# pettni/smooth_feedback

Measured on AMD Instinct MI355X. Metric: QP solves/sec, higher is better.
Workload: dtype f64

## Files before the change

include/sfb.h:

```cpp
#ifndef SFB_H
#define SFB_H

#include <stdint.h>

#ifdef __cplusplus
extern "C" {
#endif

typedef enum sfb_status {
  SFB_OK              = 0,
  SFB_ERR_INVALID_ARG = 1,
  SFB_ERR_UNSUPPORTED = 2,
  SFB_ERR_HIP         = 3,
  SFB_ERR_NO_DEVICE   = 4
} sfb_status;

typedef enum sfb_qp_status {
  SFB_QP_OPTIMAL           = 0,
  SFB_QP_POLISH_FAILED     = 1,
  SFB_QP_PRIMAL_INFEASIBLE = 2,
  SFB_QP_DUAL_INFEASIBLE   = 3,
  SFB_QP_MAX_ITERATIONS    = 4,
  SFB_QP_MAX_TIME          = 5,
  SFB_QP_UNKNOWN           = 6
// ... 64 lines not shown
                                         const double *P, const double *q, const double *A, const double *l,
                                         const double *u, const double *warm_x, const double *warm_y,
                                         double *x, double *y, double *obj, uint32_t *iter, int32_t *code);
void sfb_host_staging_trim(void);
sfb_status sfb_qp_dense_solve_batch_host_trace(const sfb_qp_params *prm, int64_t batch, int n, int m, const double *P,
                                               const double *q, const double *A, const double *l, const double *u,
                                               const double *warm_x, const double *warm_y, double *x, double *y, double *obj,
                                               uint32_t *iter, int32_t *code, double *trace, int32_t trace_rows);
sfb_status sfb_qp_dense_solve_batch_host_phases(const sfb_qp_params *prm, int64_t batch, int n, int m, const double *P,
                                                const double *q, const double *A, const double *l, const double *u,
                                                const double *warm_x, const double *warm_y, double *x, double *y, double *obj,
                                                uint32_t *iter, int32_t *code, double *trace, int32_t trace_rows,
                                                double *phase_us);
sfb_status sfb_qp_dense_solve_batch_host_multi(const sfb_qp_params *prm, int64_t batch, int n, int m,
                                               const double *P, const double *q, const double *A, const double *l,
                                               const double *u, const double *warm_x, const double *warm_y,
                                               double *x, double *y, double *obj, uint32_t *iter, int32_t *code);

#define SFB_QP_DENSE_TALL_MAX_N 16
#define SFB_QP_DENSE_TALL_MAX_M 1048576
sfb_status sfb_qp_dense_tall_solve_batch(const sfb_qp_params *prm, int64_t batch, int n, int m, const double *P,
                                         const double *q, const double *A, const double *l, const double *u,
                                         const double *warm_x, const double *warm_y, double *x, double *y,
                                         double *obj, uint32_t *iter, int32_t *code, void *stream);
sfb_status sfb_qp_dense_tall_solve_batch_host(const sfb_qp_params *prm, int64_t batch, int n, int m,
                                              const double *P, const double *q, const double *A, const double *l,
                                              const double *u, const double *warm_x, const double *warm_y,
                                              double *x, double *y, double *obj, uint32_t *iter, int32_t *code);
sfb_status sfb_qp_dense_tall_solve_batch_host_multi(const sfb_qp_params *prm, int64_t batch, int n, int m,
                                                    const double *P, const double *q, const double *A, const double *l,
                                                    const double *u, const double *warm_x, const double *warm_y,
                                                    double *x, double *y, double *obj, uint32_t *iter, int32_t *code);

typedef struct sfb_sparse_qp_plan sfb_sparse_qp_plan;

sfb_status sfb_sparse_qp_plan_create(int n, int m, const int32_t *P_colptr, const int32_t *P_rowind,
                                     const int32_t *A_rowptr, const int32_t *A_colind, int ordering,
                                     const int32_t *user_perm, sfb_sparse_qp_plan **plan);
sfb_status sfb_sparse_qp_plan_create_staged(int n, int m, const int32_t *P_colptr, const int32_t *P_rowind,
                                            const int32_t *A_rowptr, const int32_t *A_colind, int ordering,
                                            const int32_t *user_perm, const int32_t *stage,
                                            sfb_sparse_qp_plan **plan);
sfb_status sfb_sparse_qp_plan_create_pruned(int n, int m, const int32_t *P_colptr, const int32_t *P_rowind,
                                            const int32_t *A_rowptr, const int32_t *A_colind, int ordering,
                                            const int32_t *user_perm, const int32_t *stage, const uint8_t *A_keep,
                                            sfb_sparse_qp_plan **plan);
void sfb_sparse_qp_plan_destroy(sfb_sparse_qp_plan *plan);
sfb_status sfb_sparse_qp_plan_info(const sfb_sparse_qp_plan *plan, int64_t *nnzK, int64_t *nnzL,
                                   int64_t *workspace_bytes_per_item);
sfb_status sfb_sparse_qp_plan_workspace_bytes(const sfb_sparse_qp_plan *plan, int64_t batch, int64_t *bytes);
sfb_status sfb_sparse_qp_plan_pruned_info(const sfb_sparse_qp_plan *plan, int64_t *nnzA_kept, int64_t *nnzL_fallback);
sfb_status sfb_sparse_qp_plan_get_perm(const sfb_sparse_qp_plan *plan, int32_t *perm);
sfb_status sfb_sparse_qp_plan_get_factor_order(const sfb_sparse_qp_plan *plan, int fallback, int32_t *rank);

sfb_status sfb_sparse_qp_solve_batch(sfb_sparse_qp_plan *plan, const sfb_qp_params *prm, int64_t batch,
                                     const double *Px, const double *q, const double *Ax, const double *l,
                                     const double *u, const double *warm_x, const double *warm_y, double *x,
                                     double *y, double *obj, uint32_t *iter, int32_t *code, void *workspace,
                                     void *stream);
sfb_status sfb_sparse_qp_solve_batch_ordered(sfb_sparse_qp_plan *plan, const sfb_qp_params *prm, int64_t batch,
                                             const double *Px, const double *q, const double *Ax, const double *l,
                                             const double *u, const double *warm_x, const double *warm_y, double *x,
                                             double *y, double *obj, uint32_t *iter, int32_t *code, void *workspace,
                                             const int32_t *order, void *stream);
sfb_status sfb_sparse_qp_solve_batch_trace(sfb_sparse_qp_plan *plan, const sfb_qp_params *prm, int64_t batch,
                                           const double *Px, const double *q, const double *Ax, const double *l,
                                           const double *u, const double *warm_x, const double *warm_y, double *x,
                                           double *y, double *obj, uint32_t *iter, int32_t *code, void *workspace,
                                           double *trace, int32_t trace_rows, void *stream);
sfb_status sfb_sparse_qp_solve_batch_phases(sfb_sparse_qp_plan *plan, const sfb_qp_params *prm, int64_t batch,
                                            const double *Px, const double *q, const double *Ax, const double *l,
                                            const double *u, const double *warm_x, const double *warm_y, double *x,
                                            double *y, double *obj, uint32_t *iter, int32_t *code, void *workspace,
                                            double *trace, int32_t trace_rows, double *phase_us, void *stream);
sfb_status sfb_sparse_qp_solve_batch_host(sfb_sparse_qp_plan *plan, const sfb_qp_params *prm, int64_t batch,
                                          const double *Px, const double *q, const double *Ax, const double *l,
                                          const double *u, const double *warm_x, const double *warm_y,
                                          double *x, double *y, double *obj, uint32_t *iter, int32_t *code);
sfb_status sfb_sparse_qp_solve_batch_host_trace(sfb_sparse_qp_plan *plan, const sfb_qp_params *prm, int64_t batch,
                                                const double *Px, const double *q, const double *Ax, const double *l,
                                                const double *u, const double *warm_x, const double *warm_y, double *x,
                                                double *y, double *obj, uint32_t *iter, int32_t *code, double *trace,
                                                int32_t trace_rows);
sfb_status sfb_sparse_qp_solve_batch_host_phases(sfb_sparse_qp_plan *plan, const sfb_qp_params *prm, int64_t batch,
                                                 const double *Px, const double *q, const double *Ax, const double *l,
                                                 const double *u, const double *warm_x, const double *warm_y,
                                                 double *x, double *y, double *obj, uint32_t *iter, int32_t *code,
                                                 double *trace, int32_t trace_rows, double *phase_us);
sfb_status sfb_sparse_qp_solve_batch_host_multi(sfb_sparse_qp_plan *plan, const sfb_qp_params *prm, int64_t batch,
                                                const double *Px, const double *q, const double *Ax, const double *l,
                                                const double *u, const double *warm_x, const double *warm_y,
                                                double *x, double *y, double *obj, uint32_t *iter, int32_t *code);

typedef enum { SFB_LIE_RN = 0, SFB_LIE_SE2 = 1, SFB_LIE_SO3 = 2, SFB_LIE_SE3 = 3 } sfb_lie_kind;

typedef struct sfb_mpc_layout {
  int32_t nx, nu, ncr;
  int32_t kmesh, nivals;
  double tf;
  const double *alpha;
  const double *D;
  int32_t nparts;
  const int32_t *part_kind;
  const int32_t *part_dof;
  const double *crl, *cru;
  const uint8_t *jac_keep;
// ... 167 lines not shown
```

smooth_feedback_amd/_capi.py:

```python
import ctypes as C
import os

_HERE = os.path.dirname(os.path.abspath(__file__))
LIB_PATH = os.environ.get("SFB_LIB_PATH") or os.path.join(_HERE, "libsfb.so")

SFB_OK, SFB_ERR_INVALID_ARG, SFB_ERR_UNSUPPORTED, SFB_ERR_HIP, SFB_ERR_NO_DEVICE = range(5)


class SfbError(RuntimeError):
    def __init__(self, status, msg):
        super().__init__("sfb status %d: %s" % (status, msg))
        self.status = status


class SfbQPParams(C.Structure):

    _fields_ = [
        ("alpha", C.c_float),
        ("rho", C.c_float),
        ("sigma", C.c_float),
        ("scaling", C.c_int32),
        ("eps_abs", C.c_float),
        ("eps_rel", C.c_float),
        ("eps_primal_inf", C.c_float),
# ... 29 lines not shown
    _fields_ = [("nivals", C.c_int32), ("K", C.c_void_p), ("tau0", C.c_void_p)]


class SfbOcpDims(C.Structure):

    _fields_ = [("nx", C.c_int32), ("nu", C.c_int32), ("nq", C.c_int32), ("ncr", C.c_int32), ("nce", C.c_int32)]


def _load():
    if not os.path.exists(LIB_PATH):
        raise ImportError(
            "libsfb.so not found at %s: build it with `python -c 'import __graft_entry__ as g; g.build()'` "
            "or `make -C smooth_feedback_amd/csrc` (there is no CPU fallback)" % LIB_PATH)
    try:
        import torch
    except Exception:
        pass
    L = C.CDLL(LIB_PATH)
    vp, dp, i64, i32 = C.c_void_p, C.c_void_p, C.c_int64, C.c_int
    L.sfb_version.restype = C.c_char_p
    L.sfb_last_error.restype = C.c_char_p
    L.sfb_debug_set.argtypes = [C.c_char_p, C.c_char_p]
    L.sfb_device_count.argtypes = [C.POINTER(C.c_int)]
    L.sfb_qp_params_default.argtypes = [C.POINTER(SfbQPParams)]
    L.sfb_qp_params_default.restype = None
    L.sfb_qp_dense_solve_batch.argtypes = [C.POINTER(SfbQPParams), i64, i32, i32] + [dp] * 12 + [vp]
    L.sfb_qp_dense_solve_batch_host.argtypes = [C.POINTER(SfbQPParams), i64, i32, i32] + [dp] * 12
    L.sfb_qp_dense_solve_batch_host_multi.argtypes = L.sfb_qp_dense_solve_batch_host.argtypes
    L.sfb_qp_dense_tall_solve_batch.argtypes = L.sfb_qp_dense_solve_batch.argtypes
    L.sfb_qp_dense_tall_solve_batch_host.argtypes = L.sfb_qp_dense_solve_batch_host.argtypes
    L.sfb_qp_dense_tall_solve_batch_host_multi.argtypes = L.sfb_qp_dense_solve_batch_host.argtypes
    L.sfb_qp_dense_solve_batch_host_trace.argtypes = [C.POINTER(SfbQPParams), i64, i32, i32] + [dp] * 12 + [dp, i32]
    L.sfb_qp_dense_solve_batch_trace.argtypes = [C.POINTER(SfbQPParams), i64, i32, i32] + [dp] * 12 + [dp, i32, vp]
    L.sfb_qp_dense_solve_batch_host_phases.argtypes = [C.POINTER(SfbQPParams), i64, i32, i32] + [dp] * 12 + [dp, i32, dp]
    L.sfb_qp_dense_solve_batch_phases.argtypes = [C.POINTER(SfbQPParams), i64, i32, i32] + [dp] * 12 + [dp, i32, dp, vp]
    L.sfb_qp_dense_solve_batch_ws.argtypes = [C.POINTER(SfbQPParams), i64, i32, i32] + [dp] * 12 + [vp, vp]
    L.sfb_qp_dense_workspace_bytes.argtypes = [C.POINTER(SfbQPParams), i64, i32, i32, C.POINTER(C.c_int64)]
    L.sfb_workspace_create.argtypes = [i64, C.POINTER(C.c_void_p)]
    L.sfb_workspace_destroy.argtypes = [C.c_void_p]
    L.sfb_workspace_destroy.restype = None
    L.sfb_workspace_info.argtypes = [C.c_void_p, C.POINTER(C.c_void_p), C.POINTER(C.c_int64)]
    i32p = C.c_void_p
    L.sfb_sparse_qp_plan_create.argtypes = [i32, i32, i32p, i32p, i32p, i32p, i32, i32p, C.POINTER(C.c_void_p)]
    L.sfb_sparse_qp_plan_create_staged.argtypes = [i32, i32, i32p, i32p, i32p, i32p, i32, i32p, i32p, C.POINTER(C.c_void_p)]
    L.sfb_sparse_qp_plan_create_pruned.argtypes = [i32, i32, i32p, i32p, i32p, i32p, i32, i32p, i32p, C.c_void_p,
                                                   C.POINTER(C.c_void_p)]
    L.sfb_sparse_qp_plan_workspace_bytes.argtypes = [C.c_void_p, i64, C.POINTER(C.c_int64)]
    L.sfb_sparse_qp_plan_pruned_info.argtypes = [C.c_void_p, C.POINTER(C.c_int64), C.POINTER(C.c_int64)]
    L.sfb_sparse_qp_plan_destroy.argtypes = [C.c_void_p]
    L.sfb_sparse_qp_plan_destroy.restype = None
    L.sfb_sparse_qp_plan_info.argtypes = [C.c_void_p, C.POINTER(C.c_int64), C.POINTER(C.c_int64), C.POINTER(C.c_int64)]
    L.sfb_sparse_qp_plan_get_perm.argtypes = [C.c_void_p, i32p]
    L.sfb_sparse_qp_plan_get_factor_order.argtypes = [C.c_void_p, i32, i32p]
    L.sfb_sparse_qp_solve_batch.argtypes = [C.c_void_p, C.POINTER(SfbQPParams), i64] + [dp] * 12 + [vp, vp]
    L.sfb_sparse_qp_solve_batch_ordered.argtypes = [C.c_void_p, C.POINTER(SfbQPParams), i64] + [dp] * 12 + [vp, vp, vp]
    L.sfb_sparse_qp_solve_batch_host.argtypes = [C.c_void_p, C.POINTER(SfbQPParams), i64] + [dp] * 12
    L.sfb_sparse_qp_solve_batch_host_multi.argtypes = L.sfb_sparse_qp_solve_batch_host.argtypes
    L.sfb_sparse_qp_solve_batch_host_trace.argtypes = [C.c_void_p, C.POINTER(SfbQPParams), i64] + [dp] * 12 + [dp, i32]
    L.sfb_sparse_qp_solve_batch_trace.argtypes = [C.c_void_p, C.POINTER(SfbQPParams), i64] + [dp] * 12 + [vp, dp, i32, vp]
    L.sfb_sparse_qp_solve_batch_host_phases.argtypes = [C.c_void_p, C.POINTER(SfbQPParams), i64] + [dp] * 12 + [dp, i32, dp]
    L.sfb_sparse_qp_solve_batch_phases.argtypes = [C.c_void_p, C.POINTER(SfbQPParams), i64] + [dp] * 12 + [vp, dp, i32, dp, vp]
    L.sfb_ekf_predict_batch.argtypes = [i64, i32, dp, dp, i32, dp, i32, dp, vp]
    L.sfb_ekf_predict_stepper_batch.argtypes = [i32, i64, i32, dp, dp, i32, dp, i32, dp, vp]
    L.sfb_ekf_predict_stepper_batch_host.argtypes = [i32, i64, i32, dp, dp, i32, dp, i32, dp]
    L.sfb_ekf_predict_rk4_batch.argtypes = [i64, i32, dp, dp, dp, dp, i32, dp, i32, dp, vp]
    L.sfb_ekf_predict_rk4_batch_host.argtypes = [i64, i32, dp, dp, dp, dp, i32, dp, i32, dp]
    L.sfb_ekf_update_batch.argtypes = [i64, i32, i32, dp, dp, i32, dp, dp, dp, dp, vp]
    L.sfb_ekf_predict_update_batch.argtypes = [i64, i32, i32, dp, dp, i32, dp, i32, dp, dp, i32, dp, dp, dp, dp, vp]
    L.sfb_ekf_step_batch_host.argtypes = [i64, i32, i32, dp, dp, i32, dp, i32, dp, dp, i32, dp, dp, dp, dp]
    grp, dbl = C.POINTER(SfbPIDGroup), C.c_double
    L.sfb_pid_elem_doubles.argtypes = [grp]
    L.sfb_pid_elem_doubles.restype = i64
    L.sfb_pid_dof.argtypes = [grp]
    L.sfb_pid_dof.restype = i64
    L.sfb_pid_step_batch_host.argtypes = [grp, i64, dbl] + [dp] * 5 + [i32] + [dp] * 3 + [i32, dbl] + [dp] * 3
    L.sfb_pid_step_batch.argtypes = L.sfb_pid_step_batch_host.argtypes + [vp]
    L.sfb_pid_rollout_batch_host.argtypes = [grp, i64, dbl, dbl, i64] + [dp] * 4 + [i32] + [dp] * 3 + [i32, dbl] + [dp] * 5
    L.sfb_pid_rollout_batch.argtypes = L.sfb_pid_rollout_batch_host.argtypes + [vp]
    L.sfb_spline_fit_cubic_batch_host.argtypes = [grp, i64, i64, dp, i32, dp, dp]
    L.sfb_spline_fit_cubic_batch.argtypes = L.sfb_spline_fit_cubic_batch_host.argtypes + [vp]
    L.sfb_spline_eval_batch_host.argtypes = [grp, i64, i64, dp, dp, dp, i32, dp, i64, dp, i32, dp, dp, dp]
    L.sfb_spline_eval_batch.argtypes = L.sfb_spline_eval_batch_host.argtypes + [vp]
    L.sfb_pid_rollout_spline_batch_host.argtypes = [grp, i64, dbl, dbl, i64, dp, dp, i64, dp, dp, dp, i32, dp] + [dp] * 3 + [i32, dbl] + [dp] * 5
    L.sfb_pid_rollout_spline_batch.argtypes = L.sfb_pid_rollout_spline_batch_host.argtypes + [vp]
    mesh = C.POINTER(SfbMesh)
    L.sfb_mesh_raised_nodes.argtypes = [mesh, dp]
    L.sfb_mesh_resample_batch_host.argtypes = [mesh, i64, i32, i32, dp, dp]
    L.sfb_mesh_resample_batch.argtypes = L.sfb_mesh_resample_batch_host.argtypes + [vp]
    L.sfb_mesh_dyn_error_batch_host.argtypes = [mesh, i64, i32, dp, dp, dp, dp]
    L.sfb_mesh_dyn_error_batch.argtypes = L.sfb_mesh_dyn_error_batch_host.argtypes + [vp]
    L.sfb_mesh_eval_pattern.argtypes = [mesh, i32, i32, i32, vp, vp, C.POINTER(C.c_int64)]
    L.sfb_mesh_dyn_pattern.argtypes = [mesh, i32, i32, vp, vp, C.POINTER(C.c_int64)]
    L.sfb_mesh_eval_batch_host.argtypes = [mesh, i64, i32, i32, i32, i32] + [dp] * 6
    L.sfb_mesh_eval_batch.argtypes = L.sfb_mesh_eval_batch_host.argtypes + [vp]
    L.sfb_mesh_integrate_batch_host.argtypes = [mesh, i64, i32, i32, i32] + [dp] * 6
    L.sfb_mesh_integrate_batch.argtypes = L.sfb_mesh_integrate_batch_host.argtypes + [vp]
    L.sfb_mesh_dyn_batch_host.argtypes = [mesh, i64, i32, i32] + [dp] * 7
    L.sfb_mesh_dyn_batch.argtypes = L.sfb_mesh_dyn_batch_host.argtypes + [vp]
    dims = C.POINTER(SfbOcpDims)
    L.sfb_ocp_nlp_structure.argtypes = [mesh, dims, vp, vp]
    L.sfb_ocp_nlp_pattern.argtypes = [mesh, dims, vp, vp, C.POINTER(C.c_int64)]
    L.sfb_ocp_nlp_bounds.argtypes = [mesh, dims] + [dp] * 8 + [C.POINTER(C.c_double)]
    L.sfb_ocp_nlp_batch_host.argtypes = [mesh, dims, i64] + [dp] * 11
    L.sfb_ocp_nlp_batch.argtypes = L.sfb_ocp_nlp_batch_host.argtypes + [vp]
    lay = C.POINTER(SfbMPCLayout)
    L.sfb_mpc_record_doubles.argtypes = [lay, i32]
# ... 61 lines not shown
```

smooth_feedback_amd/csrc/capi_sparse.hip:

```cpp
#include <hip/hip_runtime.h>

#include <algorithm>
#include <chrono>
#include <cstdio>
#include <map>
#include <mutex>
#include <string>
#include <vector>

#include "../../include/sfb.h"
#include "capi_common.h"
#include "qp_sparse_kernel.h"
#include "sparse_plan.h"

struct sfb_sparse_qp_plan {
  sfb::SparsePlanHost host;
  bool pruned = false;
  sfb::SparsePlanHost full;
  std::vector<int32_t> Aorig, Amasked;
  std::mutex mu;
  struct DevCopy {
    int32_t *blob = nullptr, *blob_full = nullptr;
    sfb::SparsePlanDev dev{}, dev_full{};
  };
// ... 227 lines not shown
  for (auto &kv : plan->per_device) {
    if (kv.second.blob) (void)hipFree(kv.second.blob);
    if (kv.second.blob_full) (void)hipFree(kv.second.blob_full);
  }
  for (auto &kv : plan->host_dev) {
    if (kv.second.ws.first) (void)hipFree(kv.second.ws.first);
    if (kv.second.stream) (void)hipStreamDestroy(kv.second.stream);
    if (kv.second.uploaded) (void)hipEventDestroy(kv.second.uploaded);
  }
  delete plan;
}

sfb_status sfb_sparse_qp_plan_info(const sfb_sparse_qp_plan *plan, int64_t *nnzK, int64_t *nnzL,
                                   int64_t *workspace_bytes_per_item)
{
  if (!plan) return sfb::fail(SFB_ERR_INVALID_ARG, "plan is NULL");
  if (nnzK) *nnzK = plan->host.nnzK;
  if (nnzL) *nnzL = plan->host.nnzL;
  if (workspace_bytes_per_item) {
    const WsLayout L1 = ws_layout(plan, 1);
    *workspace_bytes_per_item = (int64_t)L1.total;
  }
  return SFB_OK;
}

sfb_status sfb_sparse_qp_plan_workspace_bytes(const sfb_sparse_qp_plan *plan, int64_t batch, int64_t *bytes)
{
  if (!plan || !bytes) return sfb::fail(SFB_ERR_INVALID_ARG, "NULL argument");
  if (batch < 0) return sfb::fail(SFB_ERR_INVALID_ARG, "batch < 0");
  *bytes = (int64_t)ws_layout(plan, batch).total;
  return SFB_OK;
}

sfb_status sfb_sparse_qp_plan_pruned_info(const sfb_sparse_qp_plan *plan, int64_t *nnzA_kept, int64_t *nnzL_fallback)
{
  if (!plan) return sfb::fail(SFB_ERR_INVALID_ARG, "plan is NULL");
  if (nnzA_kept) *nnzA_kept = plan->host.nnzA;
  if (nnzL_fallback) *nnzL_fallback = plan->pruned ? plan->full.nnzL : plan->host.nnzL;
  return SFB_OK;
}

sfb_status sfb_sparse_qp_plan_get_perm(const sfb_sparse_qp_plan *plan, int32_t *perm)
{
  if (!plan || !perm) return sfb::fail(SFB_ERR_INVALID_ARG, "NULL argument");
  std::copy(plan->host.perm.begin(), plan->host.perm.end(), perm);
  return SFB_OK;
}

sfb_status sfb_sparse_qp_plan_get_factor_order(const sfb_sparse_qp_plan *plan, int fallback, int32_t *rank)
{
  if (!plan || !rank) return sfb::fail(SFB_ERR_INVALID_ARG, "NULL argument");
  const sfb::SparsePlanHost &h = (fallback && plan->pruned) ? plan->full : plan->host;
  for (int f = 0; f < h.k; ++f) rank[h.f2s[f]] = f;
  return SFB_OK;
}

namespace {
sfb_status solve_batch_impl(sfb_sparse_qp_plan *plan, const sfb_qp_params *prm, int64_t batch,
                                     const double *Px, const double *q, const double *Ax, const double *l,
                                     const double *u, const double *warm_x, const double *warm_y, double *x,
                                     double *y, double *obj, uint32_t *iter, int32_t *code, void *workspace,
                                             const int32_t *order, void *stream, double *trace, int32_t trace_rows,
                                             double *phase_us = nullptr)
{
  sfb_status st = check_sparse_args(plan, prm, batch, Px, q, Ax, l, u, warm_x, warm_y, x, y, code);
  if (st != SFB_OK) return st;
  if (batch > 0 && !workspace) return sfb::fail(SFB_ERR_INVALID_ARG, "workspace is NULL");
  st = sfb::require_device();
  if (st != SFB_OK) return st;
  if (batch == 0) return SFB_OK;
  const sfb_sparse_qp_plan::DevCopy *dc = nullptr;
  st = plan_on_device(plan, &dc);
  if (st != SFB_OK) return st;
  const sfb::DenseKernelParams kp = sfb::make_kernel_params(prm, plan->host.n, plan->host.m);
  hipStream_t hs   = static_cast<hipStream_t>(stream);
  const WsLayout L = ws_layout(plan, batch);
  char *wsc        = static_cast<char *>(workspace);
  hipError_t e     = sfb::qp_sparse_launch(dc->dev, kp, batch, Px, q, Ax, l, u, warm_x, warm_y, x, y, obj, iter, code,
                                           reinterpret_cast<double *>(wsc), hs, order, reinterpret_cast<int32_t *>(wsc + L.aux_off),
                                           plan->pruned ? &dc->dev_full : nullptr, reinterpret_cast<double *>(wsc + L.pool_off),
                                           trace, (int)trace_rows, phase_us);
  if (e != hipSuccess) return sfb::hip_fail(e, "qp_sparse_kernel launch");
  return SFB_OK;
}
}

sfb_status sfb_sparse_qp_solve_batch_ordered(sfb_sparse_qp_plan *plan, const sfb_qp_params *prm, int64_t batch,
                                             const double *Px, const double *q, const double *Ax, const double *l,
                                             const double *u, const double *warm_x, const double *warm_y, double *x,
                                             double *y, double *obj, uint32_t *iter, int32_t *code, void *workspace,
                                             const int32_t *order, void *stream)
{
  return solve_batch_impl(plan, prm, batch, Px, q, Ax, l, u, warm_x, warm_y, x, y, obj, iter, code, workspace, order, stream,
                          nullptr, 0);
}

sfb_status sfb_sparse_qp_solve_batch_trace(sfb_sparse_qp_plan *plan, const sfb_qp_params *prm, int64_t batch,
                                           const double *Px, const double *q, const double *Ax, const double *l,
                                           const double *u, const double *warm_x, const double *warm_y, double *x,
                                           double *y, double *obj, uint32_t *iter, int32_t *code, void *workspace,
                                           double *trace, int32_t trace_rows, void *stream)
{
  if (!trace || trace_rows <= 0) return sfb::fail(SFB_ERR_INVALID_ARG, "trace is NULL or trace_rows <= 0");
  return solve_batch_impl(plan, prm, batch, Px, q, Ax, l, u, warm_x, warm_y, x, y, obj, iter, code, workspace, nullptr, stream,
                          trace, trace_rows);
}
// ... 203 lines not shown
```

smooth_feedback_amd/csrc/knobs.cpp:

```cpp
#include "knobs.h"

#include <atomic>
#include <cstdio>
#include <cstring>
#include <deque>
#include <map>
#include <mutex>
#include <string>

namespace sfb {

namespace {
const char *const kKnobs[] = {"SFB_SP_GRID",  "SFB_SP_SLICE",  "SFB_SP_PAUSE",      "SFB_SP_PREDICT",   "SFB_SP_LAT",
                              "SFB_SP_FORCE_LAT", "SFB_SP_LAT_WAVES", "SFB_SP_POLISHERS", "SFB_SP_LAT_HELP", "SFB_SP_PHASED", "SFB_SP_LEAN_WAVES", "SFB_MID_GRID", "SFB_MID_SLICE",
                              "SFB_QP4_MAX_WAVES", "SFB_QP_DENSE_BIG", "SFB_EKF_PERSISTENT", "SFB_PLAN_UNITS", "SFB_PLAN_DEBUG", "SFB_MPC_TIMING", "SFB_NLP_AGENTS"};
std::mutex g_mu;
std::atomic<int> g_set{0};
std::map<std::string, const char *> &table()
{
  static std::map<std::string, const char *> t;
  return t;
}
const char *intern(const char *value)
{
  static std::deque<std::string> pool;
  for (const auto &v : pool)
    if (v == value) return v.c_str();
  pool.emplace_back(value);
  return pool.back().c_str();
}
}

const char *knob(const char *name)
{
  if (g_set.load(std::memory_order_acquire) == 0) return nullptr;
  std::lock_guard<std::mutex> lk(g_mu);
  const auto &t = table();
  const auto it = t.find(name);
  return it == t.end() ? nullptr : it->second;
}

int knob_set(const char *name, const char *value)
{
  if (name == nullptr) return 1;
  bool known = false;
  for (const char *k : kKnobs) known = known || std::strcmp(k, name) == 0;
  if (!known) return 1;
  std::lock_guard<std::mutex> lk(g_mu);
  if (value == nullptr) {
    table().erase(name);
    g_set.store((int)table().size(), std::memory_order_release);
  } else {
    table()[name] = intern(value);
    g_set.store((int)table().size(), std::memory_order_release);
    std::fprintf(stderr, "[sfb] debug knob %s=%s set through sfb_debug_set (tests and measurements only; results do not depend on it)\n",
                 name, value);
  }
  return 0;
}

}
```

smooth_feedback_amd/csrc/sparse_plan.cpp:

```cpp
#include "knobs.h"
#include "sparse_plan.h"

#include <algorithm>
#include <cstdio>
#include <cstdlib>
#include <iterator>
#include <array>
#include <numeric>
#include <tuple>

namespace sfb {

namespace {

void transpose_pattern(int nouter, int ninner, const std::vector<int32_t> &outer_ptr,
                       const std::vector<int32_t> &inner, std::vector<int32_t> &tp, std::vector<int32_t> &ti,
                       std::vector<int32_t> &tpos)
{
  const int nnz = outer_ptr[nouter];
  tp.assign(ninner + 1, 0);
  ti.resize(nnz);
  tpos.resize(nnz);
  for (int p = 0; p < nnz; ++p) tp[inner[p] + 1]++;
  for (int i = 0; i < ninner; ++i) tp[i + 1] += tp[i];
// ... 162 lines not shown
      }
    }
    return {before, after};
  }
};

std::vector<int32_t> min_degree_order(int k, const std::vector<std::pair<int, int>> &edges, const int32_t *stage)
{
  const int W = (k + 63) / 64;
  std::vector<uint64_t> adj((size_t)k * W, 0);
  auto set  = [&](int a, int b) { adj[(size_t)a * W + (b >> 6)] |= (1ull << (b & 63)); };
  for (auto [a, b] : edges)
    if (a != b) { set(a, b); set(b, a); }
  std::vector<int> deg(k);
  std::vector<char> done(k, 0);
  auto degree = [&](int a) {
    int d = 0;
    for (int w = 0; w < W; ++w) d += __builtin_popcountll(adj[(size_t)a * W + w]);
    return d;
  };
  for (int a = 0; a < k; ++a) deg[a] = degree(a);
  std::vector<int32_t> order;
  order.reserve(k);
  std::vector<int> nb;
  for (int step = 0; step < k; ++step) {
    int best = -1;
    for (int a = 0; a < k; ++a) {
      if (done[a]) continue;
      if (best < 0) { best = a; continue; }
      const int sa = stage ? stage[a] : 0, sb = stage ? stage[best] : 0;
      if (sa < sb || (sa == sb && deg[a] < deg[best])) best = a;
    }
    order.push_back(best);
    done[best] = 1;
    nb.clear();
    for (int w = 0; w < W; ++w) {
      uint64_t bits = adj[(size_t)best * W + w];
      while (bits) {
        const int b = (w << 6) + __builtin_ctzll(bits);
        bits &= bits - 1;
        nb.push_back(b);
      }
    }
    for (int a : nb) {
      uint64_t *ra = &adj[(size_t)a * W];
      const uint64_t *rb = &adj[(size_t)best * W];
      for (int w = 0; w < W; ++w) ra[w] |= rb[w];
      ra[a >> 6] &= ~(1ull << (a & 63));
      ra[best >> 6] &= ~(1ull << (best & 63));
    }
    for (int a : nb) deg[a] = degree(a);
  }
  return order;
}

}

bool build_sparse_plan(int n, int m, const int32_t *Pp, const int32_t *Pi, const int32_t *Ap, const int32_t *Aj,
                       int ordering, const int32_t *user_perm, const int32_t *stage, SparsePlanHost &o,
                       const char **msg, int lds_hint)
{
  static const char *ok = "";
  *msg = ok;
  if (n < 1 || m < 1 || !Pp || !Ap) { *msg = "bad sizes / NULL pattern"; return false; }
  const int k = n + m;
  o = SparsePlanHost();
  o.n = n; o.m = m; o.k = k;
  o.nnzP = Pp[n]; o.nnzA = Ap[m];
  if (Pp[0] != 0 || Ap[0] != 0 || o.nnzP < 0 || o.nnzA < 0) { *msg = "pattern pointers must start at 0"; return false; }
  if ((o.nnzP > 0 && !Pi) || (o.nnzA > 0 && !Aj)) { *msg = "NULL index array"; return false; }
  o.Pp.assign(Pp, Pp + n + 1); o.Pi.assign(Pi, Pi + o.nnzP);
  o.Ap.assign(Ap, Ap + m + 1); o.Aj.assign(Aj, Aj + o.nnzA);
  o.Pcol.resize(o.nnzP); o.Arow.resize(o.nnzA);
  for (int c = 0; c < n; ++c) {
    if (Pp[c + 1] < Pp[c]) { *msg = "P column pointers not monotone"; return false; }
    for (int p = Pp[c]; p < Pp[c + 1]; ++p) {
      if (Pi[p] < 0 || Pi[p] >= n) { *msg = "P row index out of range"; return false; }
      if (p > Pp[c] && Pi[p] <= Pi[p - 1]) { *msg = "P row indices must be strictly ascending per column"; return false; }
      o.Pcol[p] = c;
    }
  }
  for (int r = 0; r < m; ++r) {
    if (Ap[r + 1] < Ap[r]) { *msg = "A row pointers not monotone"; return false; }
    for (int p = Ap[r]; p < Ap[r + 1]; ++p) {
      if (Aj[p] < 0 || Aj[p] >= n) { *msg = "A column index out of range"; return false; }
      if (p > Ap[r] && Aj[p] <= Aj[p - 1]) { *msg = "A column indices must be strictly ascending per row"; return false; }
      o.Arow[p] = r;
    }
  }
  transpose_pattern(m, n, o.Ap, o.Aj, o.Acp, o.Aci, o.Acpos);
  transpose_pattern(n, n, o.Pp, o.Pi, o.Prp, o.Prj, o.Prpos);

  {
    o.Sp.assign(n + 1, 0);
    for (int c = 0; c < n; ++c)
      for (int p = Pp[c]; p < Pp[c + 1]; ++p) {
        const int r = Pi[p];
        if (c >= r) { o.Sp[r + 1]++; if (r != c) o.Sp[c + 1]++; }
      }
    for (int i = 0; i < n; ++i) o.Sp[i + 1] += o.Sp[i];
    o.Sj.resize(o.Sp[n]); o.Spos.resize(o.Sp[n]);
    std::vector<int32_t> fill(n, 0);
    for (int c = 0; c < n; ++c)
      for (int p = Pp[c]; p < Pp[c + 1]; ++p)
        if (Pi[p] < c) { o.Sj[o.Sp[c] + fill[c]] = Pi[p]; o.Spos[o.Sp[c] + fill[c]] = p; fill[c]++; }
    for (int c = 0; c < n; ++c)
// ... 614 lines not shown
        heap.emplace_back(height[q], -q);
        std::push_heap(heap.begin(), heap.end());
      }
    }
    const int steps = (int)slots.size();
    if (const char *dbg = sfb::knob("SFB_PLAN_DEBUG"); dbg && dbg[0] == '1') {
      fprintf(stderr, "[sfb plan] %s sweep: %d units, slots per unit:", forward ? "forward" : "backward", steps);
      for (int s = 0; s < steps; ++s) fprintf(stderr, " %d", (int)slots[s].size());
      fprintf(stderr, "\n");
    }
    units           = steps;
    units = ((units + 7) / 8) * 8;
    const size_t total = (size_t)(units + SparsePlanHost::kSweepPad) * 128;
    xmap.assign(total, -1);
    const int sc = o.idx_scale;
    xidx.assign(total, (k * sc) | ((k * sc) << 16));
    xmask.assign((size_t)units + 2 * SparsePlanHost::kSweepPad, 63);
    constexpr bool bank_aware = true;
    long cyc_before = 0, cyc_after = 0;
    UnitPlacer up;
    const int search_passes = ns <= 20000 ? 1 : 0;
    for (int s = 0; s < steps; ++s) {
      const int lanes = std::max(1, ((int)slots[s].size() + 1) / 2);
      xmask[s]        = 64 - lanes;
      up.lanes = lanes;
      up.sl.clear();
      for (const auto &e : slots[s]) up.sl.push_back({e[1], e[2]});
      const auto cyc = up.place(search_passes);
      cyc_before += cyc.first;
      cyc_after += bank_aware ? cyc.second : cyc.first;
      for (size_t e = 0; e < slots[s].size(); ++e) {
        const int pos  = bank_aware ? up.where[e] : (int)((e % (size_t)lanes) * 2 + e / (size_t)lanes);
        const size_t q = (size_t)s * 128 + (size_t)pos;
        xmap[q] = acc_of(slots[s][e][0]);
        xidx[q] = (slots[s][e][1] * sc) | ((slots[s][e][2] * sc) << 16);
      }
    }
    if (const char *dbg = sfb::knob("SFB_PLAN_DEBUG"); dbg && dbg[0] == '1')
      fprintf(stderr, "[sfb plan] %s sweep: modelled LDS cycles of the slot accesses per sweep: natural placement %ld, bank-aware %ld (floor %d)\n",
              forward ? "forward" : "backward", cyc_before, cyc_after, 16 * steps);
    full0 = full1 = 0;
    for (int s = 0; s < steps;) {
      if ((int)slots[s].size() != cap) { ++s; continue; }
      int e = s;
      while (e < steps && (int)slots[e].size() == cap) ++e;
      const int a = ((s + 7) / 8) * 8, b = (e / 8) * 8;
      if (b - a > full1 - full0) { full0 = a; full1 = b; }
      s = e;
    }
  };
  build(true, o.fmap, o.fidx, o.funits, o.fmask, o.ffull0, o.ffull1);
  build(false, o.bmap, o.bidx, o.bunits, o.bmask, o.bfull0, o.bfull1);

  return true;
}

}
```

smooth_feedback_amd/csrc/sparse_plan.h:

```cpp
#pragma once
#include <cstdint>
#include <vector>

namespace sfb {

#ifndef SFB_KKT_KINDS
#define SFB_KKT_KINDS
enum { K_P = 0, K_A = 1, K_SIGMA = 2, K_RHO = 3 };
#endif

struct SparsePlanHost {
  int n = 0, m = 0, k = 0, nnzP = 0, nnzA = 0, nnzK = 0, nnzL = 0;
  std::vector<int32_t> Pp, Pi, Pcol;
  std::vector<int32_t> Ap, Aj, Arow;
  std::vector<int32_t> Acp, Aci, Acpos;
  std::vector<int32_t> Prp, Prj, Prpos;
  std::vector<int32_t> Sp, Sj, Spos;
  std::vector<int32_t> perm, pinv;
  std::vector<int32_t> Kp, Ki, Kkind, Kidx;
  std::vector<int32_t> Lp, Li;
  std::vector<int32_t> Rp, Rk, Rpos;
  std::vector<int32_t> Rlen;
  static constexpr int kSweepPad = 16;
  std::vector<int32_t> fmap, fidx, bmap, bidx, fmask, bmask;
  int funits = 0, bunits = 0, idx_scale = 1, ffull0 = 0, ffull1 = 0, bfull0 = 0, bfull1 = 0;
  std::vector<int32_t> Kmap, rptr, rtgt, rab, snptr, snR, poff, pmap;
  std::vector<int32_t> Kdesc;
  int rsteps = 0, maxcol = 0, nsn = 0, lds_doubles = 0;
  std::vector<int32_t> f2s;
  static constexpr int kSegStride = 12;
  std::vector<int32_t> seg, pmapL, rsplit, KmapL, KdescT, KmapT, ztop;
  int nseg = 0, nnzKT = 0, nztop = 0;
  std::vector<int32_t> ustream, utype, uomap;
  int units = 0, nunits = 0;
};

bool build_sparse_plan(int n, int m, const int32_t *Pp, const int32_t *Pi, const int32_t *Ap, const int32_t *Aj,
                       int ordering, const int32_t *user_perm, const int32_t *stage, SparsePlanHost &out,
                       const char **msg, int lds_hint = 0);

}
```

smooth_feedback_amd/qp.py:

```python
import ctypes as C
import enum
from dataclasses import dataclass, field
from typing import Optional

import numpy as np

from . import _capi


class QPSolutionStatus(enum.IntEnum):
    Optimal = 0
    PolishFailed = 1
    PrimalInfeasible = 2
    DualInfeasible = 3
    MaxIterations = 4
    MaxTime = 5
    Unknown = 6


@dataclass
class QPSolverParams:
    verbose: bool = False
    alpha: float = 1.6
    rho: float = 0.1
# ... 260 lines not shown


class SparseQPPlan:

    def __init__(self, n, m, P_colptr, P_rowind, A_rowptr, A_colind, ordering=1, user_perm=None, stage=None,
                 keep=None):
        self.n, self.m = int(n), int(m)
        self._keep = [np.ascontiguousarray(a, dtype=np.int32) for a in (P_colptr, P_rowind, A_rowptr, A_colind)]
        up = None if user_perm is None else np.ascontiguousarray(user_perm, dtype=np.int32)
        st = None if stage is None else np.ascontiguousarray(stage, dtype=np.int32)
        if st is not None and st.shape != (self.n + self.m,):
            raise ValueError("stage must have n+m entries")
        kp = None
        if keep is not None:
            kp = np.ascontiguousarray(np.asarray(keep) != 0, dtype=np.uint8)
            if kp.shape != (int(self._keep[2][-1]),):
                raise ValueError("keep must have nnzA entries")
        h = C.c_void_p()
        _capi.check(_capi.lib.sfb_sparse_qp_plan_create_pruned(
            self.n, self.m, *[_ptr(a) if a.size else None for a in self._keep], int(ordering), _ptr(up), _ptr(st),
            _ptr(kp), C.byref(h)))
        self._h = h
        a, b, c_ = C.c_int64(), C.c_int64(), C.c_int64()
        _capi.check(_capi.lib.sfb_sparse_qp_plan_info(h, C.byref(a), C.byref(b), C.byref(c_)))
        self.nnzK, self.nnzL, self.workspace_bytes_per_item = a.value, b.value, c_.value
        self.nnzP, self.nnzA = int(self._keep[0][-1]), int(self._keep[2][-1])
        _capi.check(_capi.lib.sfb_sparse_qp_plan_pruned_info(h, C.byref(a), C.byref(b)))
        self.nnzA_kept, self.nnzL_fallback = a.value, b.value
        self.pruned = self.nnzA_kept != self.nnzA

    def workspace_bytes(self, batch):
        v = C.c_int64()
        _capi.check(_capi.lib.sfb_sparse_qp_plan_workspace_bytes(self._h, int(batch), C.byref(v)))
        return v.value

    @classmethod
    def from_scipy(cls, P, A, **kw):
        import scipy.sparse as sp
        P = sp.csc_matrix(P); P.sort_indices()
        A = sp.csr_matrix(A); A.sort_indices()
        return cls(A.shape[1], A.shape[0], P.indptr, P.indices, A.indptr, A.indices, **kw)

    @property
    def perm(self):
        p = np.empty(self.n + self.m, dtype=np.int32)
        _capi.check(_capi.lib.sfb_sparse_qp_plan_get_perm(self._h, _ptr(p)))
        return p

    def factor_order(self, fallback=False):
        r = np.empty(self.n + self.m, dtype=np.int32)
        _capi.check(_capi.lib.sfb_sparse_qp_plan_get_factor_order(self._h, int(bool(fallback)), _ptr(r)))
        return r

    def close(self):
        if getattr(self, "_h", None):
            _capi.lib.sfb_sparse_qp_plan_destroy(self._h)
            self._h = None

    def __del__(self):
        try:
            self.close()
        except Exception:
            pass

    def solve_batch_host(self, Px, q, Ax, l, u, prm: Optional[QPSolverParams] = None, warm_x=None, warm_y=None,
                         multi_device=False, trace_rows=0, phases=False, out: Optional["QPBatchSolution"] = None):
        q = np.ascontiguousarray(q, dtype=np.float64)
        B = q.shape[0]
        Px = _f64(np.reshape(Px, (B, self.nnzP)), (B, self.nnzP))
        Ax = _f64(np.reshape(Ax, (B, self.nnzA)), (B, self.nnzA))
        q = _f64(q, (B, self.n)); l = _f64(l, (B, self.m)); u = _f64(u, (B, self.m))
        if (warm_x is None) != (warm_y is None):
            raise ValueError("warm_x and warm_y must be given together")
        if warm_x is not None:
            warm_x = _f64(warm_x, (B, self.n)); warm_y = _f64(warm_y, (B, self.m))
        if out is not None:
            x, y, obj, it, code = out.primal, out.dual, out.objective, out.iter, out.code
            for a, shp, dt in ((x, (B, self.n), np.float64), (y, (B, self.m), np.float64), (obj, (B,), np.float64),
                               (it, (B,), np.uint32), (code, (B,), np.int32)):
                if a.shape != shp or a.dtype != dt or not a.flags.c_contiguous or not a.flags.writeable:
                    raise ValueError("out: arrays of another batch size or layout")
        else:
            x = np.empty((B, self.n)); y = np.empty((B, self.m)); obj = np.empty(B)
            it = np.empty(B, dtype=np.uint32); code = np.empty(B, dtype=np.int32)
        cp = (prm or QPSolverParams()).to_c()
        if trace_rows or phases:
            if multi_device:
                raise ValueError("trace_rows / phases and multi_device exclude each other")
            trace = np.empty((B, int(trace_rows), 5)) if trace_rows else None
            ph = np.zeros((B, 6)) if phases else None
            _capi.check(_capi.lib.sfb_sparse_qp_solve_batch_host_phases(
                self._h, C.byref(cp), B, _ptr(Px), _ptr(q), _ptr(Ax), _ptr(l), _ptr(u), _ptr(warm_x), _ptr(warm_y),
                _ptr(x), _ptr(y), _ptr(obj), _ptr(it), _ptr(code), _ptr(trace), int(trace_rows), _ptr(ph)))
            return QPBatchSolution(code=code, iter=it, primal=x, dual=y, objective=obj, trace=trace, phase_us=ph)
        fn = _capi.lib.sfb_sparse_qp_solve_batch_host_multi if multi_device else _capi.lib.sfb_sparse_qp_solve_batch_host
        _capi.check(fn(
            self._h, C.byref(cp), B, _ptr(Px), _ptr(q), _ptr(Ax), _ptr(l), _ptr(u), _ptr(warm_x), _ptr(warm_y),
            _ptr(x), _ptr(y), _ptr(obj), _ptr(it), _ptr(code)))
        return QPBatchSolution(code=code, iter=it, primal=x, dual=y, objective=obj)

    def solve_batch_device(self, B, dPx, dq, dAx, dl, du, dx, dy, dobj, diter, dcode, dworkspace, prm=None,
                           dwarm_x=0, dwarm_y=0, stream=0, dorder=0):
        cp = (prm or QPSolverParams()).to_c()
        _capi.check(_capi.lib.sfb_sparse_qp_solve_batch_ordered(
            self._h, C.byref(cp), B, dPx, dq, dAx, dl, du, dwarm_x or None, dwarm_y or None, dx, dy,
            dobj or None, diter or None, dcode, dworkspace, dorder or None, stream or None))
# ... 26 lines not shown
```

Before: 224,500.

## Reorder factor storage per segment to cut modelled memory sectors in sweeps

```diff
diff --git a/include/sfb.h b/include/sfb.h
--- a/include/sfb.h
+++ b/include/sfb.h
@@ -140,6 +140,8 @@
 sfb_status sfb_sparse_qp_plan_pruned_info(const sfb_sparse_qp_plan *plan, int64_t *nnzA_kept, int64_t *nnzL_fallback);
 sfb_status sfb_sparse_qp_plan_get_perm(const sfb_sparse_qp_plan *plan, int32_t *perm);
 sfb_status sfb_sparse_qp_plan_get_factor_order(const sfb_sparse_qp_plan *plan, int fallback, int32_t *rank);
+sfb_status sfb_sparse_qp_plan_copy_stats(const sfb_sparse_qp_plan *plan, int fallback, int64_t *sectors, int64_t *lines,
+                                         int32_t *layout, uint64_t *sweep_hash);
 
 sfb_status sfb_sparse_qp_solve_batch(sfb_sparse_qp_plan *plan, const sfb_qp_params *prm, int64_t batch,
                                      const double *Px, const double *q, const double *Ax, const double *l,
diff --git a/smooth_feedback_amd/_capi.py b/smooth_feedback_amd/_capi.py
--- a/smooth_feedback_amd/_capi.py
+++ b/smooth_feedback_amd/_capi.py
@@ -105,6 +105,7 @@
     L.sfb_sparse_qp_plan_info.argtypes = [C.c_void_p, C.POINTER(C.c_int64), C.POINTER(C.c_int64), C.POINTER(C.c_int64)]
     L.sfb_sparse_qp_plan_get_perm.argtypes = [C.c_void_p, i32p]
     L.sfb_sparse_qp_plan_get_factor_order.argtypes = [C.c_void_p, i32, i32p]
+    L.sfb_sparse_qp_plan_copy_stats.argtypes = [C.c_void_p, i32, i32p, i32p, C.POINTER(C.c_int32), C.POINTER(C.c_uint64)]
     L.sfb_sparse_qp_solve_batch.argtypes = [C.c_void_p, C.POINTER(SfbQPParams), i64] + [dp] * 12 + [vp, vp]
     L.sfb_sparse_qp_solve_batch_ordered.argtypes = [C.c_void_p, C.POINTER(SfbQPParams), i64] + [dp] * 12 + [vp, vp, vp]
     L.sfb_sparse_qp_solve_batch_host.argtypes = [C.c_void_p, C.POINTER(SfbQPParams), i64] + [dp] * 12
diff --git a/smooth_feedback_amd/csrc/capi_sparse.hip b/smooth_feedback_amd/csrc/capi_sparse.hip
--- a/smooth_feedback_amd/csrc/capi_sparse.hip
+++ b/smooth_feedback_amd/csrc/capi_sparse.hip
@@ -303,6 +303,21 @@
   if (!plan || !rank) return sfb::fail(SFB_ERR_INVALID_ARG, "NULL argument");
   const sfb::SparsePlanHost &h = (fallback && plan->pruned) ? plan->full : plan->host;
   for (int f = 0; f < h.k; ++f) rank[h.f2s[f]] = f;
+  return SFB_OK;
+}
+
+sfb_status sfb_sparse_qp_plan_copy_stats(const sfb_sparse_qp_plan *plan, int fallback, int64_t *sectors, int64_t *lines,
+                                         int32_t *layout, uint64_t *sweep_hash)
+{
+  if (!plan) return sfb::fail(SFB_ERR_INVALID_ARG, "plan is NULL");
+  const sfb::SparsePlanHost &h = (fallback && plan->pruned) ? plan->full : plan->host;
+  for (int v = 0; v < 2; ++v)
+    for (int a = 0; a < 4; ++a) {
+      if (sectors) sectors[4 * v + a] = h.traffic_sectors[v][a];
+      if (lines) lines[4 * v + a] = h.traffic_lines[v][a];
+    }
+  if (layout) *layout = h.layout;
+  if (sweep_hash) *sweep_hash = h.sweep_hash;
   return SFB_OK;
 }
 
diff --git a/smooth_feedback_amd/csrc/knobs.cpp b/smooth_feedback_amd/csrc/knobs.cpp
--- a/smooth_feedback_amd/csrc/knobs.cpp
+++ b/smooth_feedback_amd/csrc/knobs.cpp
@@ -13,7 +13,7 @@
 namespace {
 const char *const kKnobs[] = {"SFB_SP_GRID",  "SFB_SP_SLICE",  "SFB_SP_PAUSE",      "SFB_SP_PREDICT",   "SFB_SP_LAT",
                               "SFB_SP_FORCE_LAT", "SFB_SP_LAT_WAVES", "SFB_SP_POLISHERS", "SFB_SP_LAT_HELP", "SFB_SP_PHASED", "SFB_SP_LEAN_WAVES", "SFB_MID_GRID", "SFB_MID_SLICE",
-                              "SFB_QP4_MAX_WAVES", "SFB_QP_DENSE_BIG", "SFB_EKF_PERSISTENT", "SFB_PLAN_UNITS", "SFB_PLAN_DEBUG", "SFB_MPC_TIMING", "SFB_NLP_AGENTS"};
+                              "SFB_QP4_MAX_WAVES", "SFB_QP_DENSE_BIG", "SFB_EKF_PERSISTENT", "SFB_PLAN_UNITS", "SFB_PLAN_LAYOUT", "SFB_PLAN_DEBUG", "SFB_MPC_TIMING", "SFB_NLP_AGENTS"};
 std::mutex g_mu;
 std::atomic<int> g_set{0};
 std::map<std::string, const char *> &table()
diff --git a/smooth_feedback_amd/csrc/sparse_plan.cpp b/smooth_feedback_amd/csrc/sparse_plan.cpp
--- a/smooth_feedback_amd/csrc/sparse_plan.cpp
+++ b/smooth_feedback_amd/csrc/sparse_plan.cpp
@@ -238,6 +238,240 @@
     for (int a : nb) deg[a] = degree(a);
   }
   return order;
+}
+
+struct SectorCount {
+  std::vector<int32_t> sec, lin;
+  int32_t stamp = 0;
+  int ns = 0, nl = 0;
+  explicit SectorCount(int nacc) : sec((size_t)nacc / 8 + 1, 0), lin((size_t)nacc / 16 + 1, 0) {}
+  void begin() { ++stamp; ns = nl = 0; }
+  void touch(int a)
+  {
+    if (sec[a >> 3] != stamp) { sec[a >> 3] = stamp; ++ns; }
+    if (lin[a >> 4] != stamp) { lin[a >> 4] = stamp; ++nl; }
+  }
+};
+
+constexpr int kOmapBatch = 8;
+
+void omap_traffic(const SparsePlanHost &o, const std::vector<int32_t> &uomap, SectorCount &sc, int64_t res[2][2])
+{
+  res[0][0] = res[0][1] = res[1][0] = res[1][1] = 0;
+  if (!o.units) return;
+  for (int s = 0; s < o.nseg; ++s) {
+    const int nout = o.seg[(size_t)SparsePlanHost::kSegStride * s + 10], omap0 = o.seg[(size_t)SparsePlanHost::kSegStride * s + 11];
+    for (int b0 = 0; b0 < nout; b0 += 64 * kOmapBatch) {
+      const int active = std::min(64, nout - b0);
+      for (int e = 0; e < kOmapBatch; ++e) {
+        sc.begin();
+        for (int lane = 0; lane < active; ++lane) sc.touch(uomap[(size_t)omap0 + b0 + e * 64 + lane]);
+        res[0][0] += sc.ns; res[0][1] += sc.nl;
+        sc.begin();
+        for (int lane = 0; lane < 64 && b0 + e * 64 + lane < nout; ++lane) sc.touch(uomap[(size_t)omap0 + b0 + e * 64 + lane]);
+        res[1][0] += sc.ns; res[1][1] += sc.nl;
+      }
+    }
+  }
+}
+
+uint64_t fnv1a(uint64_t h, const int32_t *p, size_t n)
+{
+  for (size_t i = 0; i < n; ++i)
+    for (int b = 0; b < 4; ++b) h = (h ^ (uint64_t)(((uint32_t)p[i] >> (8 * b)) & 0xFFu)) * 1099511628211ull;
+  return h;
+}
+
+void lay_out_factor(SparsePlanHost &o)
+{
+  constexpr int SS = SparsePlanHost::kSegStride;
+  const int nnzL = o.nnzL, nacc = o.nnzL + o.k + 2, ZERO = o.nnzL + o.k + 1;
+  {
+    uint64_t h = 1469598103934665603ull;
+    for (const std::vector<int32_t> *v : {&o.fidx, &o.bidx, &o.fmask, &o.bmask}) h = fnv1a(h, v->data(), v->size());
+    const int32_t sc[6] = {o.funits, o.bunits, o.ffull0, o.ffull1, o.bfull0, o.bfull1};
+    o.sweep_hash = fnv1a(h, sc, 6);
+  }
+  o.apos.resize((size_t)nacc);
+  std::iota(o.apos.begin(), o.apos.end(), 0);
+  o.layout = 0;
+  std::vector<int32_t> &apos = o.apos;
+  SectorCount sc(nacc);
+
+  const std::vector<int32_t> *maps[2] = {&o.fmap, &o.bmap};
+  std::vector<int32_t> cntS[2], cntL[2], slot[2];
+  int64_t tot[2] = {0, 0};
+  auto instr = [&](const int dir, const int i) {
+    const int32_t *mp = maps[dir]->data() + (size_t)i * 64;
+    sc.begin();
+    for (int lane = 0; lane < 64; ++lane) sc.touch(mp[lane] < 0 ? ZERO : apos[mp[lane]]);
+  };
+  for (int dir = 0; dir < 2; ++dir) {
+    const int ni = (int)(maps[dir]->size() / 64);
+    cntS[dir].resize((size_t)ni); cntL[dir].resize((size_t)ni);
+    slot[dir].assign((size_t)nnzL, 0);
+    for (size_t q = 0; q < maps[dir]->size(); ++q)
+      if ((*maps[dir])[q] >= 0) slot[dir][(*maps[dir])[q]] = (int32_t)q;
+    for (int i = 0; i < ni; ++i) {
+      instr(dir, i);
+      cntS[dir][i] = sc.ns; cntL[dir][i] = sc.nl;
+      tot[dir] += sc.ns;
+      o.traffic_lines[0][dir] += sc.nl;
+    }
+    o.traffic_sectors[0][dir] = tot[dir];
+  }
+  int64_t om[2][2];
+  omap_traffic(o, o.uomap, sc, om);
+  for (int a = 0; a < 2; ++a) { o.traffic_sectors[0][2 + a] = om[a][0]; o.traffic_lines[0][2 + a] = om[a][1]; }
+  for (int a = 0; a < 4; ++a) { o.traffic_sectors[1][a] = o.traffic_sectors[0][a]; o.traffic_lines[1][a] = o.traffic_lines[0][a]; }
+  const char *lk = sfb::knob("SFB_PLAN_LAYOUT");
+  const bool dbg = [] { const char *d = sfb::knob("SFB_PLAN_DEBUG"); return d && d[0] == '1'; }();
+  auto report = [&] {
+    if (!dbg) return;
+    static const char *const name[4] = {"forward copy", "backward copy", "outside accumulators in", "outside accumulators out"};
+    for (int a = 0; a < 4; ++a)
+      fprintf(stderr, "[sfb plan] layout: %s: modelled 64-byte sectors %lld column-major, %lld chosen; 128-byte lines %lld, %lld\n", name[a],
+              (long long)o.traffic_sectors[0][a], (long long)o.traffic_sectors[1][a], (long long)o.traffic_lines[0][a], (long long)o.traffic_lines[1][a]);
+  };
+  if (lk && lk[0] == '0') { report(); return; }
+
+  std::vector<int32_t> ord, keep, ins[2], newS[2], newL[2];
+  std::vector<uint32_t> key;
+  auto morton = [](uint32_t x, uint32_t y) {
+    uint32_t r = 0;
+    for (int b = 0; b < 16; ++b) r |= ((x >> b) & 1u) << (2 * b) | ((y >> b) & 1u) << (2 * b + 1);
+    return r;
+  };
+  int chosen_count[4] = {0, 0, 0, 0};
+  for (int s = 0; s < o.nseg; ++s) {
+    const int gL = o.seg[(size_t)SS * s + 9], nL = (s + 1 < o.nseg ? o.seg[(size_t)SS * (s + 1) + 9] : nnzL) - gL;
+    if (nL < 2) continue;
+    for (int dir = 0; dir < 2; ++dir) {
+      ins[dir].clear();
+      for (int g = gL; g < gL + nL; ++g) ins[dir].push_back(slot[dir][g] / 64);
+      std::sort(ins[dir].begin(), ins[dir].end());
+      ins[dir].erase(std::unique(ins[dir].begin(), ins[dir].end()), ins[dir].end());
+    }
+    keep.assign(apos.begin() + gL, apos.begin() + gL + nL);
+    int64_t best = tot[0] + tot[1];
+    int best_cand = -1;
+    auto place = [&](const int cand) {
+      if (cand < 0) { std::copy(keep.begin(), keep.end(), apos.begin() + gL); return; }
+      ord.resize((size_t)nL);
+      key.resize((size_t)nL);
+      std::iota(ord.begin(), ord.end(), 0);
+      for (int e = 0; e < nL; ++e) {
+        const uint32_t f = (uint32_t)slot[0][gL + e], b = (uint32_t)slot[1][gL + e];
+        const int tile = cand == 2 ? 1 : cand == 3 ? 4 : 16;
+        key[e] = cand == 0 ? f : cand == 1 ? b : morton(f / 128 / tile, b / 128 / tile);
+      }
+      std::sort(ord.begin(), ord.end(), [&](int x, int y) {
+        return key[x] != key[y] ? key[x] < key[y] : slot[0][gL + x] < slot[0][gL + y];
+      });
+      for (int i = 0; i < nL; ++i) apos[gL + ord[i]] = gL + i;
+    };
+    auto measure = [&](int64_t t2[2]) {
+      for (int dir = 0; dir < 2; ++dir) {
+        newS[dir].resize(ins[dir].size()); newL[dir].resize(ins[dir].size());
+        t2[dir] = tot[dir];
+        for (size_t x = 0; x < ins[dir].size(); ++x) {
+          instr(dir, ins[dir][x]);
+          newS[dir][x] = sc.ns; newL[dir][x] = sc.nl;
+          t2[dir] += sc.ns - cntS[dir][ins[dir][x]];
+        }
+      }
+    };
+    for (int cand = 0; cand < 5; ++cand) {
+      place(cand);
+      int64_t t2[2];
+      measure(t2);
+      if (t2[0] <= o.traffic_sectors[0][0] && t2[1] <= o.traffic_sectors[0][1] && t2[0] + t2[1] < best) { best = t2[0] + t2[1]; best_cand = cand; }
+    }
+    place(best_cand);
+    int64_t t2[2];
+    measure(t2);
+    for (int dir = 0; dir < 2; ++dir) {
+      tot[dir] = t2[dir];
+      for (size_t x = 0; x < ins[dir].size(); ++x) { cntS[dir][ins[dir][x]] = newS[dir][x]; cntL[dir][ins[dir][x]] = newL[dir][x]; }
+    }
+    if (best_cand >= 0) chosen_count[std::min(best_cand, 2)]++;
+    else chosen_count[3]++;
+  }
+
+  std::vector<int32_t> uomap, rank;
+  auto order_omap = [&](const bool sorted) {
+    uomap = o.uomap;
+    rank.assign(o.uomap.size(), 0);
+    if (!o.units) return;
+    std::vector<std::pair<int32_t, int32_t>> tmp;
+    for (int s = 0; s < o.nseg; ++s) {
+      const int nout = o.seg[(size_t)SS * s + 10], omap0 = o.seg[(size_t)SS * s + 11];
+      tmp.clear();
+      for (int e = 0; e < nout; ++e) tmp.emplace_back(apos[o.uomap[(size_t)omap0 + e]], e);
+      if (sorted) std::sort(tmp.begin(), tmp.end());
+      for (int e = 0; e < nout; ++e) { uomap[(size_t)omap0 + e] = tmp[e].first; rank[(size_t)omap0 + tmp[e].second] = e; }
+    }
+  };
+  bool found = false;
+  for (int attempt = 0; attempt < 3 && !found; ++attempt) {
+    if (attempt == 2) {
+      std::iota(apos.begin(), apos.end(), 0);
+      tot[0] = o.traffic_sectors[0][0]; tot[1] = o.traffic_sectors[0][1];
+    }
+    order_omap(attempt != 1);
+    omap_traffic(o, uomap, sc, om);
+    found = om[0][0] <= o.traffic_sectors[0][2] && om[1][0] <= o.traffic_sectors[0][3];
+  }
+  if (!found) { report(); return; }
+  bool identity = uomap == o.uomap;
+  for (int g = 0; g < nnzL && identity; ++g) identity = apos[g] == g;
+  if (identity) { report(); return; }
+  o.layout = 1;
+  for (int dir = 0; dir < 2; ++dir) {
+    o.traffic_sectors[1][dir] = o.traffic_lines[1][dir] = 0;
+    for (size_t i = 0; i < cntS[dir].size(); ++i) {
+      instr(dir, (int)i);
+      o.traffic_sectors[1][dir] += sc.ns; o.traffic_lines[1][dir] += sc.nl;
+    }
+  }
+  for (int a = 0; a < 2; ++a) { o.traffic_sectors[1][2 + a] = om[a][0]; o.traffic_lines[1][2 + a] = om[a][1]; }
+  if (dbg)
+    fprintf(stderr, "[sfb plan] layout: segments by forward slot %d, by backward slot %d, tiled %d, column-major %d\n", chosen_count[0],
+            chosen_count[1], chosen_count[2], chosen_count[3]);
+  report();
+
+  auto A = [&](int32_t &g) { if (g >= 0) g = apos[g]; };
+  for (std::vector<int32_t> *v : {&o.fmap, &o.bmap, &o.Kmap, &o.KmapT, &o.pmap}) for (int32_t &g : *v) A(g);
+  for (int s = 0; s < o.nseg; ++s) {
+    const int32_t *sg = o.seg.data() + (size_t)SS * s;
+    const int gL = sg[9], nL = (s + 1 < o.nseg ? sg[SS + 9] : nnzL) - gL, accN = sg[6], nout = sg[10], omap0 = sg[11];
+    auto own = [&](const int x) { return x < nL ? apos[gL + x] - gL : x; };
+    if (sg[4])
+      for (int p = sg[7]; p < sg[8]; ++p) o.KmapL[p] = own(o.KmapL[p]);
+    if (o.units) {
+      auto off = [&](const uint32_t b) -> uint32_t {
+        const int x = (int)(b / 8);
+        if (x < accN) return (uint32_t)own(x) * 8;
+        if (x < accN + nout) return (uint32_t)(accN + rank[(size_t)omap0 + (x - accN)]) * 8;
+        return b;
+      };
+      auto word = [&](int32_t &w) { const uint32_t u = (uint32_t)w; w = (int32_t)(off(u & 0xFFFFu) | off(u >> 16) << 16); };
+      for (int u = sg[0]; u < sg[1]; ++u)
+        for (int e = 0; e < 128; ++e) {
+          int32_t *w = o.ustream.data() + (size_t)u * 256 + (size_t)e * 2;
+          word(w[0]);
+          if (!o.utype[u]) word(w[1]);
+        }
+    } else {
+      for (int sn = sg[0]; sn < sg[1]; ++sn) {
+        if (sg[4])
+          for (int q = o.poff[sn]; q < o.poff[sn + 1]; ++q) o.pmapL[q] = own(o.pmapL[q]);
+        for (int q = o.rptr[sn] * 64; q < o.rsplit[sn] * 64; ++q) o.rtgt[q] = own(o.rtgt[q]);
+        for (int q = o.rsplit[sn] * 64; q < o.rptr[sn + 1] * 64; ++q) A(o.rtgt[q]);
+      }
+    }
+  }
+  o.uomap.swap(uomap);
 }
 
 }
@@ -958,6 +1192,7 @@
   build(true, o.fmap, o.fidx, o.funits, o.fmask, o.ffull0, o.ffull1);
   build(false, o.bmap, o.bidx, o.bunits, o.bmask, o.bfull0, o.bfull1);
 
+  lay_out_factor(o);
   return true;
 }
 
diff --git a/smooth_feedback_amd/csrc/sparse_plan.h b/smooth_feedback_amd/csrc/sparse_plan.h
--- a/smooth_feedback_amd/csrc/sparse_plan.h
+++ b/smooth_feedback_amd/csrc/sparse_plan.h
@@ -33,6 +33,10 @@
   int nseg = 0, nnzKT = 0, nztop = 0;
   std::vector<int32_t> ustream, utype, uomap;
   int units = 0, nunits = 0;
+  std::vector<int32_t> apos;
+  int layout = 0;
+  int64_t traffic_sectors[2][4] = {{0, 0, 0, 0}, {0, 0, 0, 0}}, traffic_lines[2][4] = {{0, 0, 0, 0}, {0, 0, 0, 0}};
+  uint64_t sweep_hash = 0;
 };
 
 bool build_sparse_plan(int n, int m, const int32_t *Pp, const int32_t *Pi, const int32_t *Ap, const int32_t *Aj,
diff --git a/smooth_feedback_amd/qp.py b/smooth_feedback_amd/qp.py
--- a/smooth_feedback_amd/qp.py
+++ b/smooth_feedback_amd/qp.py
@@ -336,6 +336,13 @@
         _capi.check(_capi.lib.sfb_sparse_qp_plan_get_factor_order(self._h, int(bool(fallback)), _ptr(r)))
         return r
 
+    def copy_stats(self, fallback=False):
+        sec, lin = np.zeros((2, 4), dtype=np.int64), np.zeros((2, 4), dtype=np.int64)
+        lay, h = C.c_int32(0), C.c_uint64(0)
+        _capi.check(_capi.lib.sfb_sparse_qp_plan_copy_stats(self._h, int(bool(fallback)), _ptr(sec), _ptr(lin), C.byref(lay),
+                                                            C.byref(h)))
+        return {"sectors": sec, "lines": lin, "layout": lay.value, "sweep_hash": h.value}
+
     def close(self):
         if getattr(self, "_h", None):
             _capi.lib.sfb_sparse_qp_plan_destroy(self._h)
```

Result: no change. 226,600 (median of 6 runs) (+0.9%).
